# Zehong-Ma/MagCache

Measured on NVIDIA H100. Metric: denoising_steps_per_sec, higher is better.
Workload: dtype bf16

## Files before the change

### magcache_b200/csrc/attn_wgmma.cu

```cuda
#include <cstdlib>

#include "common.cuh"
#include "ptx.cuh"
#include "tma_host.cuh"

#ifndef MC_ATTN_EMU_DEFAULT
#define MC_ATTN_EMU_DEFAULT 0
#endif

namespace mc {

constexpr int kHD = 128;
constexpr int kLongMinLk = 1024;

struct AttnParams {
  int Lq, Lk, heads;
  int q_blocks, full_units, tail_units, tail_split;
  float* part_o;
  float2* part_ml;
  float scale_log2;
  __nv_bfloat16* out;
  int64_t ldo;
  int tile_rot;
  const uint32_t* seg_flags;
  const uint32_t* seg_epoch;
  int seg_rows;
};

struct WorkItem {
  int q_block, head;
  int split, nsplit;
  int tail_unit;
};

__device__ __forceinline__ WorkItem work_item(const AttnParams& p) {
  WorkItem w;
  int c = blockIdx.x, unit;
  if (c < p.full_units) {
    unit = c, w.split = 0, w.nsplit = 1, w.tail_unit = 0;
  } else {
    c -= p.full_units;
    w.tail_unit = c / p.tail_split;
    w.split = c - w.tail_unit * p.tail_split;
    w.nsplit = p.tail_split;
    unit = p.full_units + w.tail_unit;
  }
  w.head = unit / p.q_blocks;
  w.q_block = unit - w.head * p.q_blocks;
  return w;
}

template <uint32_t EMU_MASK>
__device__ __forceinline__ float exp2_sel(float x, int group) {
  return ((EMU_MASK >> (group & 7)) & 1u) ? ptx::ex2_emul(x) : ptx::ex2_approx(x);
}

__device__ __forceinline__ void wait_segments(const AttnParams& p, int row0, int rows) {
  if (p.seg_flags == nullptr) return;
  const uint32_t want = *reinterpret_cast<const volatile uint32_t*>(p.seg_epoch);
  const int last = min(row0 + rows, p.Lk) - 1;
  const int s0 = row0 / p.seg_rows, s1 = last / p.seg_rows;
  for (int s = s0; s <= s1; ++s) {
    const uint32_t* f = p.seg_flags + s;
    const long long t0 = clock64();
    for (;;) {
      uint32_t v;
      asm volatile("ld.acquire.sys.global.u32 %0, [%1];" : "=r"(v) : "l"(f) : "memory");
      if (static_cast<int32_t>(v - want) >= 0) break;
      __nanosleep(100);
      if (clock64() - t0 > MC_MBAR_TIMEOUT_CYCLES) {
        MC_DIAG("attention: key segment %d never arrived (flag %u, epoch %u)\n", s, v, want);
        __trap();
      }
    }
  }
  asm volatile("fence.proxy.async;" ::: "memory");
}

namespace ak {
constexpr int kBQ = 128;
constexpr int kQBytes = kBQ * kHD * 2;
constexpr int kThreads = 384;
constexpr int kProducerRegs = 24, kConsumerRegs = 240;
template <int BKV>
struct Layout {
  static constexpr int kKBytes = BKV * kHD * 2;
  static constexpr int kVBytes = BKV * kHD * 2;
  static constexpr int kOffK = kQBytes;
  static constexpr int kOffV = kOffK + 2 * kKBytes;
  static constexpr int kOffBar = kOffV + 2 * kVBytes;
  static constexpr int kSmem = kOffBar + 128;
};
}

template <int BKV, uint32_t EMU_MASK>
__global__ void __launch_bounds__(ak::kThreads, 1)
    attn_kernel(const __grid_constant__ CUtensorMap tmap_q, const __grid_constant__ CUtensorMap tmap_k,
                const __grid_constant__ CUtensorMap tmap_v, const AttnParams p) {
  using namespace ak;
  using L = Layout<BKV>;
  extern __shared__ __align__(1024) uint8_t smem[];
  uint64_t* bars = reinterpret_cast<uint64_t*>(smem + L::kOffBar);
  uint64_t* q_full = bars + 0;
  uint64_t* k_full = bars + 1;
  uint64_t* k_empty = bars + 3;
  uint64_t* v_full = bars + 5;
  uint64_t* v_empty = bars + 7;

  const int warp = threadIdx.x >> 5, lane = threadIdx.x & 31;
  const WorkItem wi = work_item(p);
  const int q0 = wi.q_block * kBQ;
  const int head = wi.head;
  const int total_tiles = (p.Lk + BKV - 1) / BKV;
  const int per_split = (total_tiles + wi.nsplit - 1) / wi.nsplit;
  const int t0 = wi.split * per_split;
  const int n_tiles = min(per_split, total_tiles - t0);
  auto tile_of = [&](int j) {
    int t = p.tile_rot + t0 + j;
    return t >= total_tiles ? t - total_tiles : t;
  };

  if (threadIdx.x == 0) {
    if ((ptx::smem_u32(smem) & 1023u) != 0) {
      MC_DIAG("attn_kernel: dynamic smem base not 1024-aligned\n");
      __trap();
    }
    ptx::prefetch_tmap(&tmap_q);
    ptx::prefetch_tmap(&tmap_k);
    ptx::prefetch_tmap(&tmap_v);
    ptx::mbar_init(q_full, 1);
    for (int s = 0; s < 2; ++s) {
      ptx::mbar_init(&k_full[s], 1);
      ptx::mbar_init(&k_empty[s], 8);
      ptx::mbar_init(&v_full[s], 1);
      ptx::mbar_init(&v_empty[s], 8);
    }
    ptx::fence_mbar_init();
  }
  __syncthreads();

  if (warp < 4) {
    ptx::setmaxnreg_dec<kProducerRegs>();
    if (warp == 0) {
      if (ptx::elect_one()) {
        ptx::mbar_expect_tx(q_full, kQBytes);
        ptx::tma_load_2d(smem, &tmap_q, q_full, head * kHD, q0);
        ptx::tma_load_2d(smem + kQBytes / 2, &tmap_q, q_full, head * kHD + 64, q0);
      }
      __syncwarp();
      for (int j = 0; j < n_tiles; ++j) {
        const int s = j & 1;
        const uint32_t ph = (j >> 1) & 1;
        const int kv0 = tile_of(j) * BKV;
        if (p.seg_flags != nullptr) {
          if (lane == 0) wait_segments(p, kv0, BKV);
          __syncwarp();
        }
        ptx::mbar_wait(&k_empty[s], ph ^ 1);
        if (ptx::elect_one()) {
          ptx::mbar_expect_tx(&k_full[s], L::kKBytes);
          ptx::tma_load_2d(smem + L::kOffK + s * L::kKBytes, &tmap_k, &k_full[s], head * kHD, kv0);
          ptx::tma_load_2d(smem + L::kOffK + s * L::kKBytes + L::kKBytes / 2, &tmap_k, &k_full[s], head * kHD + 64, kv0);
        }
        __syncwarp();
        ptx::mbar_wait(&v_empty[s], ph ^ 1);
        if (ptx::elect_one()) {
          ptx::mbar_expect_tx(&v_full[s], L::kVBytes);
          ptx::tma_load_2d(smem + L::kOffV + s * L::kVBytes, &tmap_v, &v_full[s], head * kHD, kv0);
          ptx::tma_load_2d(smem + L::kOffV + s * L::kVBytes + L::kVBytes / 2, &tmap_v, &v_full[s], head * kHD + 64, kv0);
        }
        __syncwarp();
      }
    }
  } else {
    ptx::setmaxnreg_inc<kConsumerRegs>();
    const int wg = (warp >> 2) - 1;
    const int r = wg * 64 + (warp & 3) * 16 + (lane >> 2);
    const int cq = 2 * (lane & 3);
    const uint32_t q_base = ptx::smem_u32(smem) + wg * (64 * 128);
    const uint32_t k_base = ptx::smem_u32(smem + L::kOffK), v_base = ptx::smem_u32(smem + L::kOffV);
    int j_ragged = -1;
    if (p.Lk % BKV != 0) {
      int jr = total_tiles - 1 - p.tile_rot - t0;
      if (jr < 0) jr += total_tiles;
      if (jr < n_tiles) j_ragged = jr;
    }
    float o[kHD / 2];
#pragma unroll
    for (int i = 0; i < kHD / 2; ++i) o[i] = 0.f;
    float m0 = -INFINITY, m1 = -INFINITY, l0 = 0.f, l1 = 0.f;
    bool timed_out = false;
    ptx::mbar_wait_or_flag(q_full, 0, timed_out);

    constexpr uint32_t kTurnThreads = 256;
    const uint32_t bar_own = 1 + wg, bar_other = 2 - wg;
    auto turn_begin = [&] { ptx::named_bar_sync(bar_own, kTurnThreads); };
    auto turn_end = [&] { ptx::named_bar_arrive(bar_other, kTurnThreads); };
    if (wg == 0) ptx::named_bar_arrive(bar_own, kTurnThreads);

    float sc[BKV / 2];
    uint32_t pa[BKV / 16][4];
    const int valid = p.Lk - (total_tiles - 1) * BKV;
    auto issue_s = [&](int j) {
      const int s = j & 1;
      ptx::wgmma_fence();
#pragma unroll
      for (int kk = 0; kk < kHD / 16; ++kk) {
        const uint64_t da = ptx::gmma_desc_sw128_kmajor(q_base + (kk >> 2) * (kQBytes / 2)) + 2 * (kk & 3);
        const uint64_t db = ptx::gmma_desc_sw128_kmajor(k_base + s * L::kKBytes + (kk >> 2) * (L::kKBytes / 2)) + 2 * (kk & 3);
        if constexpr (BKV == 128) {
          ptx::wgmma_m64n128k16_ss(sc, da, db, kk != 0 ? 1u : 0u);
        } else {
          ptx::wgmma_m64n64k16_ss(sc, da, db, kk != 0 ? 1u : 0u);
        }
      }
      ptx::wgmma_commit();
    };
    auto issue_pv = [&](int j) {
      const int s = j & 1;
      ptx::fence_regs(o);
      ptx::wgmma_fence();
      const uint64_t dv = ptx::gmma_desc_sw128_mnmajor(v_base + s * L::kVBytes, BKV * 128);
#pragma unroll
      for (int kk = 0; kk < BKV / 16; ++kk)
        ptx::wgmma_m64n128k16_rs_tb(o, pa[kk], dv + static_cast<uint64_t>(kk * (2048 / 16)), 1u);
      ptx::wgmma_commit();
    };
    auto softmax = [&](int j, float& f0, float& f1) {
      ptx::fence_regs(sc);
      __syncwarp();
      if (lane == 0) ptx::mbar_arrive(&k_empty[j & 1]);
      if (j == j_ragged) {
#pragma unroll
        for (int i = 0; i < BKV / 8; ++i)
#pragma unroll
          for (int e = 0; e < 4; ++e)
            if (8 * i + cq + (e & 1) >= valid) sc[4 * i + e] = -INFINITY;
      }
      float mx0 = -INFINITY, mx1 = -INFINITY;
#pragma unroll
      for (int i = 0; i < BKV / 8; ++i) {
        mx0 = fmaxf(mx0, fmaxf(sc[4 * i], sc[4 * i + 1]));
        mx1 = fmaxf(mx1, fmaxf(sc[4 * i + 2], sc[4 * i + 3]));
      }
#pragma unroll
      for (int off = 1; off <= 2; off <<= 1) {
        mx0 = fmaxf(mx0, __shfl_xor_sync(0xffffffffu, mx0, off));
        mx1 = fmaxf(mx1, __shfl_xor_sync(0xffffffffu, mx1, off));
      }
      const float mn0 = fmaxf(m0, mx0 * p.scale_log2), mn1 = fmaxf(m1, mx1 * p.scale_log2);
      f0 = ptx::ex2_approx(m0 - mn0), f1 = ptx::ex2_approx(m1 - mn1);
      m0 = mn0, m1 = mn1;
      l0 *= f0, l1 *= f1;
#pragma unroll
      for (int i = 0; i < BKV / 8; ++i) {
        sc[4 * i] = exp2_sel<EMU_MASK>(fmaf(sc[4 * i], p.scale_log2, -m0), i);
        sc[4 * i + 1] = exp2_sel<EMU_MASK>(fmaf(sc[4 * i + 1], p.scale_log2, -m0), i);
        sc[4 * i + 2] = exp2_sel<EMU_MASK>(fmaf(sc[4 * i + 2], p.scale_log2, -m1), i);
        sc[4 * i + 3] = exp2_sel<EMU_MASK>(fmaf(sc[4 * i + 3], p.scale_log2, -m1), i);
        l0 += sc[4 * i] + sc[4 * i + 1];
        l1 += sc[4 * i + 2] + sc[4 * i + 3];
      }
    };
    auto pack_p = [&] {
#pragma unroll
      for (int i = 0; i < BKV / 8; ++i) {
        pa[i >> 1][(i & 1) * 2] = pack_bf16x2(sc[4 * i], sc[4 * i + 1]);
        pa[i >> 1][(i & 1) * 2 + 1] = pack_bf16x2(sc[4 * i + 2], sc[4 * i + 3]);
      }
    };
    auto release_v = [&](int j) {
      ptx::fence_regs(o);
      __syncwarp();
      if (lane == 0) ptx::mbar_arrive(&v_empty[j & 1]);
    };
    auto rescale_o = [&](float f0, float f1) {
#pragma unroll
      for (int i = 0; i < kHD / 8; ++i) {
        o[4 * i] *= f0, o[4 * i + 1] *= f0;
        o[4 * i + 2] *= f1, o[4 * i + 3] *= f1;
      }
    };
    {
      ptx::mbar_wait_or_flag(&k_full[0], 0, timed_out);
      turn_begin();
      issue_s(0);
      turn_end();
      ptx::wgmma_wait<0>();
      float f0, f1;
      softmax(0, f0, f1);
      rescale_o(f0, f1);
      pack_p();
    }
    for (int j = 1; j < n_tiles; ++j) {
      ptx::mbar_wait_or_flag(&k_full[j & 1], (j >> 1) & 1, timed_out);
      ptx::mbar_wait_or_flag(&v_full[(j - 1) & 1], ((j - 1) >> 1) & 1, timed_out);
      turn_begin();
      issue_s(j);
      issue_pv(j - 1);
      turn_end();
      ptx::wgmma_wait<1>();
      float f0, f1;
      softmax(j, f0, f1);
      ptx::wgmma_wait<0>();
      release_v(j - 1);
      rescale_o(f0, f1);
      pack_p();
    }
    {
      const int j = n_tiles - 1;
      ptx::mbar_wait_or_flag(&v_full[j & 1], (j >> 1) & 1, timed_out);
      turn_begin();
      issue_pv(j);
      if (wg == 0) turn_end();
      ptx::wgmma_wait<0>();
      release_v(j);
    }
    if (timed_out) __trap();

#pragma unroll
    for (int off = 1; off <= 2; off <<= 1) {
      l0 += __shfl_xor_sync(0xffffffffu, l0, off);
      l1 += __shfl_xor_sync(0xffffffffu, l1, off);
    }
    const bool partial = wi.nsplit > 1;
#pragma unroll
    for (int h = 0; h < 2; ++h) {
      const float inv_l = 1.0f / (h ? l1 : l0);
      const int rt = r + 8 * h;
      const int row = q0 + rt;
      if (row >= p.Lq) continue;
      if (partial) {
        const int64_t prow = (static_cast<int64_t>(wi.split) * p.tail_units + wi.tail_unit) * kBQ + rt;
        if ((lane & 3) == 0) p.part_ml[prow] = make_float2(h ? m1 : m0, h ? l1 : l0);
        float* dst = p.part_o + prow * kHD + cq;
#pragma unroll
        for (int i = 0; i < kHD / 8; ++i)
          *reinterpret_cast<float2*>(dst + 8 * i) = make_float2(o[4 * i + 2 * h] * inv_l, o[4 * i + 2 * h + 1] * inv_l);
      } else {
        __nv_bfloat16* dst = p.out + static_cast<int64_t>(row) * p.ldo + head * kHD + cq;
#pragma unroll
        for (int i = 0; i < kHD / 8; ++i)
          *reinterpret_cast<uint32_t*>(dst + 8 * i) = pack_bf16x2(o[4 * i + 2 * h] * inv_l, o[4 * i + 2 * h + 1] * inv_l);
      }
    }
  }
}

__global__ void __launch_bounds__(256) attn_combine_kernel(const float* __restrict__ part_o, const float2* __restrict__ part_ml, int nsplit,
                                                           int tail_units, int full_units, int q_blocks, int rows_per_cta, int Lq,
                                                           __nv_bfloat16* __restrict__ out, int64_t ldo) {
  constexpr int kGroups = kHD / 8;
  const int64_t total = static_cast<int64_t>(tail_units) * rows_per_cta * kGroups;
  const int64_t split_stride = static_cast<int64_t>(tail_units) * rows_per_cta;
  for (int64_t i = static_cast<int64_t>(blockIdx.x) * blockDim.x + threadIdx.x; i < total; i += static_cast<int64_t>(gridDim.x) * blockDim.x) {
    const int64_t prow = i / kGroups;
    const int g = static_cast<int>(i - prow * kGroups);
    const int tu = static_cast<int>(prow / rows_per_cta), r = static_cast<int>(prow - static_cast<int64_t>(tu) * rows_per_cta);
    const int unit = full_units + tu;
    const int head = unit / q_blocks, row = (unit - head * q_blocks) * rows_per_cta + r;
    if (row >= Lq) continue;
    float mmax = -INFINITY;
    for (int s = 0; s < nsplit; ++s) mmax = fmaxf(mmax, part_ml[s * split_stride + prow].x);
    float acc[8] = {0.f, 0.f, 0.f, 0.f, 0.f, 0.f, 0.f, 0.f};
    float wsum = 0.f;
    for (int s = 0; s < nsplit; ++s) {
      const float2 ml = part_ml[s * split_stride + prow];
      const float w = ml.y * ptx::ex2_approx(ml.x - mmax);
      wsum += w;
      float v[8];
      ptx::ld_nc_v8_f32(part_o + (s * split_stride + prow) * kHD + g * 8, v);
#pragma unroll
      for (int j = 0; j < 8; ++j) acc[j] = fmaf(w, v[j], acc[j]);
    }
    const float inv = 1.0f / wsum;
#pragma unroll
    for (int j = 0; j < 8; ++j) acc[j] *= inv;
    *reinterpret_cast<uint4*>(out + static_cast<int64_t>(row) * ldo + head * kHD + g * 8) = pack_bf16x8(acc);
  }
}

struct AttnPlan {
  bool long_kernel;
  int q_blocks, kv_tile, total_tiles, rows_per_cta;
  int full_units, tail_units, tail_split;
  size_t ws_bytes;
  int grid() const { return full_units + tail_units * tail_split; }
};

static int env_int(const char* name, int lo, int hi, int dflt) {
  const char* e = getenv(name);
  if (!e || !*e) return dflt;
  const int v = atoi(e);
  return (v < lo || v > hi) ? dflt : v;
}

static AttnPlan plan_attention(int Lq, int Lk, int heads, bool need_long = false) {
  AttnPlan pl;
  const int forced_splits = env_int("MC_ATTN_SPLITS", 1, 16, 0);
  const int kernel_sel = env_int("MC_ATTN_KERNEL", 0, 2, 0);
  pl.long_kernel = need_long || kernel_sel == 2 || (kernel_sel == 0 && Lk >= kLongMinLk);
  pl.rows_per_cta = ak::kBQ;
  pl.kv_tile = pl.long_kernel ? 128 : 64;
  pl.q_blocks = (Lq + pl.rows_per_cta - 1) / pl.rows_per_cta;
  pl.total_tiles = (Lk + pl.kv_tile - 1) / pl.kv_tile;
  const int64_t units = static_cast<int64_t>(pl.q_blocks) * heads;
  const int slots = num_sms();
  const int min_tiles_per_split = pl.long_kernel ? 4 : 8;
  int full = static_cast<int>(units), tail = 0, split = 1;
  if (forced_splits > 0) {
    if (forced_splits > 1) full = 0, tail = static_cast<int>(units), split = forced_splits;
  } else {
    const int rem = static_cast<int>(units % slots);
    const int by_tiles = pl.total_tiles / min_tiles_per_split;
    int f = rem > 0 ? slots / rem : 1;
    if (f > 8) f = 8;
    if (f > by_tiles) f = by_tiles;
    if (f >= 2) full = static_cast<int>(units) - rem, tail = rem, split = f;
  }
  if (split > pl.total_tiles) split = pl.total_tiles;
  if (split > 1) {
    const int per = (pl.total_tiles + split - 1) / split;
    split = (pl.total_tiles + per - 1) / per;
  }
  if (split <= 1) full = static_cast<int>(units), tail = 0, split = 1;
  pl.full_units = full, pl.tail_units = tail, pl.tail_split = split;
  pl.ws_bytes = tail > 0 ? static_cast<size_t>(split) * tail * pl.rows_per_cta * (kHD * sizeof(float) + sizeof(float2)) : 0;
  return pl;
}

}

extern "C" int32_t mc_attn_workspace_bytes(int32_t Lq, int32_t Lk, int32_t heads, int64_t* bytes_out) {
  MC_CHECK_ARG(bytes_out != nullptr && Lq >= 1 && Lk >= 1 && heads >= 1, "mc_attn_workspace_bytes: bad arguments");
  const size_t a = mc::plan_attention(Lq, Lk, heads, false).ws_bytes, b = mc::plan_attention(Lq, Lk, heads, true).ws_bytes;
  *bytes_out = static_cast<int64_t>(a > b ? a : b);
  return MC_OK;
}

extern "C" int32_t mc_attn_fwd_ex(const void* q, int64_t ldq, const void* k, int64_t ldk, const void* v, int64_t ldv, void* out,
                                  int64_t ldo, int32_t Lq, int32_t Lk, int32_t heads, float scale, void* workspace,
                                  int64_t workspace_bytes, int32_t first_key_row, const uint32_t* seg_flags, const uint32_t* seg_epoch,
                                  int32_t seg_rows, void* stream) {
  MC_CHECK_ARG(q && k && v && out, "mc_attn_fwd: null pointer");
  MC_CHECK_ARG(Lq >= 1 && Lk >= 1 && heads >= 1, "mc_attn_fwd: Lq=%d Lk=%d heads=%d", Lq, Lk, heads);
  const int64_t width = static_cast<int64_t>(heads) * mc::kHD;
  MC_CHECK_ARG(ldq >= width && ldk >= width && ldo >= width && ldv >= width, "mc_attn_fwd: leading dimensions too small");
  MC_CHECK_ARG(ldq % 8 == 0 && ldk % 8 == 0 && ldv % 8 == 0 && ldo % 8 == 0, "mc_attn_fwd: leading dimensions must be multiples of 8");
  MC_CHECK_ARG(mc::aligned16(q) && mc::aligned16(k) && mc::aligned16(v) && mc::aligned16(out), "mc_attn_fwd: pointers must be 16-byte aligned");
  MC_CHECK_ARG(first_key_row >= 0 && first_key_row < Lk, "mc_attn_fwd: first_key_row=%d outside [0, %d)", first_key_row, Lk);
  MC_CHECK_ARG(seg_flags == nullptr || (seg_rows >= 1 && seg_epoch != nullptr), "mc_attn_fwd: seg_rows=%d / null epoch", seg_rows);
  const mc::AttnPlan pl = mc::plan_attention(Lq, Lk, heads, first_key_row != 0 || seg_flags != nullptr);
  MC_CHECK_ARG(static_cast<int64_t>(pl.q_blocks) * heads * 8 < INT32_MAX, "mc_attn_fwd: grid too large");
  if (pl.tail_units > 0) {
    MC_CHECK_ARG(workspace != nullptr && workspace_bytes >= static_cast<int64_t>(pl.ws_bytes) && (reinterpret_cast<uintptr_t>(workspace) & 31u) == 0,
                 "mc_attn_fwd: split-KV needs a 32-byte aligned workspace of %lld bytes (mc_attn_workspace_bytes), got %lld",
                 static_cast<long long>(pl.ws_bytes), static_cast<long long>(workspace_bytes));
  }
  const int q_box = mc::ak::kBQ;
  CUtensorMap tq, tk, tv;
  int32_t rc = mc::make_tmap_bf16_2d(&tq, q, static_cast<uint64_t>(Lq), static_cast<uint64_t>(width), static_cast<uint64_t>(ldq), q_box, 64);
  if (rc) return rc;
  rc = mc::make_tmap_bf16_2d(&tk, k, static_cast<uint64_t>(Lk), static_cast<uint64_t>(width), static_cast<uint64_t>(ldk), pl.kv_tile, 64);
  if (rc) return rc;
  rc = mc::make_tmap_bf16_2d(&tv, v, static_cast<uint64_t>(Lk), static_cast<uint64_t>(width), static_cast<uint64_t>(ldv), pl.kv_tile, 64);
  if (rc) return rc;

  float* part_o = static_cast<float*>(workspace);
  const size_t part_rows = static_cast<size_t>(pl.tail_split) * pl.tail_units * pl.rows_per_cta;
  float2* part_ml = pl.tail_units > 0 ? reinterpret_cast<float2*>(part_o + part_rows * mc::kHD) : nullptr;
  mc::AttnParams p{};
  p.Lq = Lq, p.Lk = Lk, p.heads = heads;
  p.q_blocks = pl.q_blocks, p.full_units = pl.full_units, p.tail_units = pl.tail_units, p.tail_split = pl.tail_split;
  p.part_o = pl.tail_units > 0 ? part_o : nullptr, p.part_ml = part_ml;
  p.scale_log2 = scale * 1.4426950408889634f;
  p.out = static_cast<__nv_bfloat16*>(out), p.ldo = ldo;
  p.tile_rot = ((first_key_row + pl.kv_tile - 1) / pl.kv_tile) % pl.total_tiles;
  p.seg_flags = seg_flags, p.seg_epoch = seg_epoch, p.seg_rows = seg_rows > 0 ? seg_rows : Lk;

  dim3 grid(pl.grid(), 1, 1);
  cudaStream_t st = static_cast<cudaStream_t>(stream);
  if (pl.long_kernel) {
    static mc::PerDeviceOnce once[4];
    const int emu = mc::env_int("MC_ATTN_EMU", 0, 4, MC_ATTN_EMU_DEFAULT);
#define MC_LAUNCH_LONG(MASK, IDX)                                                                                                    \
  do {                                                                                                                               \
    rc = mc::set_max_smem_once(mc::attn_kernel<128, MASK>, mc::ak::Layout<128>::kSmem, once[IDX], "cudaFuncSetAttribute(attn smem)"); \
    if (rc) return rc;                                                                                                               \
    mc::attn_kernel<128, MASK><<<grid, mc::ak::kThreads, mc::ak::Layout<128>::kSmem, st>>>(tq, tk, tv, p);                           \
  } while (0)
    switch (emu) {
      case 2: MC_LAUNCH_LONG(0x88u, 1); break;
      case 3: MC_LAUNCH_LONG(0x92u, 2); break;
      case 4: MC_LAUNCH_LONG(0xAAu, 3); break;
      default: MC_LAUNCH_LONG(0x00u, 0); break;
    }
#undef MC_LAUNCH_LONG
  } else {
    static mc::PerDeviceOnce once;
    rc = mc::set_max_smem_once(mc::attn_kernel<64, 0u>, mc::ak::Layout<64>::kSmem, once, "cudaFuncSetAttribute(attn smem)");
    if (rc) return rc;
    mc::attn_kernel<64, 0u><<<grid, mc::ak::kThreads, mc::ak::Layout<64>::kSmem, st>>>(tq, tk, tv, p);
  }
  MC_CHECK_LAUNCH("attn_kernel launch");
  if (pl.tail_units > 0) {
    const int64_t total = static_cast<int64_t>(pl.tail_units) * pl.rows_per_cta * (mc::kHD / 8);
    const int64_t want = (total + 255) / 256, cap = static_cast<int64_t>(mc::num_sms()) * 8;
    mc::attn_combine_kernel<<<static_cast<int>(want < cap ? want : cap), 256, 0, st>>>(
        p.part_o, p.part_ml, pl.tail_split, pl.tail_units, pl.full_units, pl.q_blocks, pl.rows_per_cta, Lq, static_cast<__nv_bfloat16*>(out), ldo);
    MC_CHECK_LAUNCH("attn_combine_kernel launch");
  }
  return MC_OK;
}

extern "C" int32_t mc_attn_fwd(const void* q, int64_t ldq, const void* k, int64_t ldk, const void* v, int64_t ldv, void* out,
                               int64_t ldo, int32_t Lq, int32_t Lk, int32_t heads, float scale, void* workspace,
                               int64_t workspace_bytes, void* stream) {
  return mc_attn_fwd_ex(q, ldq, k, ldk, v, ldv, out, ldo, Lq, Lk, heads, scale, workspace, workspace_bytes, 0, nullptr, nullptr, 0, stream);
}
```

Before: 1.654.

## Multicast K/V tiles across 2-CTA clusters in long attention kernel

The long-sequence attention kernel now runs as 2-CTA clusters that handle adjacent query blocks of the same head. Each CTA loads half of every K/V tile and multicasts it to both CTAs via TMA, and empty barriers are released cluster-wide. This halves L2-to-SM K/V traffic per query block. The ring also grows to three stages, and scheduling slots are sized with cudaOccupancyMaxActiveClusters. The cost is cross-CTA synchronisation coupling, since one slow CTA stalls its partner, plus coarser work units that can hurt load balance.

```diff
diff --git a/magcache_b200/csrc/attn_wgmma.cu b/magcache_b200/csrc/attn_wgmma.cu
--- a/magcache_b200/csrc/attn_wgmma.cu
+++ b/magcache_b200/csrc/attn_wgmma.cu
@@ -15,7 +15,7 @@
 
 struct AttnParams {
   int Lq, Lk, heads;
-  int q_blocks, full_units, tail_units, tail_split;
+  int head_units, full_units, tail_units, tail_split;
   float* part_o;
   float2* part_ml;
   float scale_log2;
@@ -33,9 +33,10 @@
   int tail_unit;
 };
 
-__device__ __forceinline__ WorkItem work_item(const AttnParams& p) {
+template <int CL>
+__device__ __forceinline__ WorkItem work_item(const AttnParams& p, int rank) {
   WorkItem w;
-  int c = blockIdx.x, unit;
+  int c = static_cast<int>(blockIdx.x / CL), unit;
   if (c < p.full_units) {
     unit = c, w.split = 0, w.nsplit = 1, w.tail_unit = 0;
   } else {
@@ -45,8 +46,8 @@
     w.nsplit = p.tail_split;
     unit = p.full_units + w.tail_unit;
   }
-  w.head = unit / p.q_blocks;
-  w.q_block = unit - w.head * p.q_blocks;
+  w.head = unit / p.head_units;
+  w.q_block = (unit - w.head * p.head_units) * CL + rank;
   return w;
 }
 
@@ -82,33 +83,40 @@
 constexpr int kQBytes = kBQ * kHD * 2;
 constexpr int kThreads = 384;
 constexpr int kProducerRegs = 24, kConsumerRegs = 240;
-template <int BKV>
+constexpr int kPairStages = 3;
+template <int BKV, int CL>
 struct Layout {
+  static constexpr int kStages = CL > 1 ? kPairStages : 2;
   static constexpr int kKBytes = BKV * kHD * 2;
   static constexpr int kVBytes = BKV * kHD * 2;
+  static constexpr int kPartRows = BKV / CL;
   static constexpr int kOffK = kQBytes;
-  static constexpr int kOffV = kOffK + 2 * kKBytes;
-  static constexpr int kOffBar = kOffV + 2 * kVBytes;
+  static constexpr int kOffV = kOffK + kStages * kKBytes;
+  static constexpr int kOffBar = kOffV + kStages * kVBytes;
   static constexpr int kSmem = kOffBar + 128;
 };
-}
-
-template <int BKV, uint32_t EMU_MASK>
+#define MC_RING_STAGE(S, j) ((S) == 2 ? ((j) & 1) : ((j) % (S)))
+#define MC_RING_PHASE(S, j) ((S) == 2 ? (((j) >> 1) & 1) : (((j) / (S)) & 1))
+}
+
+template <int BKV, uint32_t EMU_MASK, int CL>
 __global__ void __launch_bounds__(ak::kThreads, 1)
     attn_kernel(const __grid_constant__ CUtensorMap tmap_q, const __grid_constant__ CUtensorMap tmap_k,
                 const __grid_constant__ CUtensorMap tmap_v, const AttnParams p) {
   using namespace ak;
-  using L = Layout<BKV>;
+  using L = Layout<BKV, CL>;
+  constexpr int S = L::kStages;
   extern __shared__ __align__(1024) uint8_t smem[];
   uint64_t* bars = reinterpret_cast<uint64_t*>(smem + L::kOffBar);
   uint64_t* q_full = bars + 0;
   uint64_t* k_full = bars + 1;
-  uint64_t* k_empty = bars + 3;
-  uint64_t* v_full = bars + 5;
-  uint64_t* v_empty = bars + 7;
+  uint64_t* k_empty = bars + 1 + S;
+  uint64_t* v_full = bars + 1 + 2 * S;
+  uint64_t* v_empty = bars + 1 + 3 * S;
 
   const int warp = threadIdx.x >> 5, lane = threadIdx.x & 31;
-  const WorkItem wi = work_item(p);
+  const int rank = CL > 1 ? static_cast<int>(ptx::cluster_ctarank()) : 0;
+  const WorkItem wi = work_item<CL>(p, rank);
   const int q0 = wi.q_block * kBQ;
   const int head = wi.head;
   const int total_tiles = (p.Lk + BKV - 1) / BKV;
@@ -129,15 +137,20 @@
     ptx::prefetch_tmap(&tmap_k);
     ptx::prefetch_tmap(&tmap_v);
     ptx::mbar_init(q_full, 1);
-    for (int s = 0; s < 2; ++s) {
+    for (int s = 0; s < S; ++s) {
       ptx::mbar_init(&k_full[s], 1);
-      ptx::mbar_init(&k_empty[s], 8);
+      ptx::mbar_init(&k_empty[s], 8 * CL);
       ptx::mbar_init(&v_full[s], 1);
-      ptx::mbar_init(&v_empty[s], 8);
+      ptx::mbar_init(&v_empty[s], 8 * CL);
     }
     ptx::fence_mbar_init();
   }
-  __syncthreads();
+  if constexpr (CL > 1) {
+    ptx::cluster_arrive();
+    ptx::cluster_wait();
+  } else {
+    __syncthreads();
+  }
 
   if (warp < 4) {
     ptx::setmaxnreg_dec<kProducerRegs>();
@@ -149,27 +162,45 @@
       }
       __syncwarp();
       for (int j = 0; j < n_tiles; ++j) {
-        const int s = j & 1;
-        const uint32_t ph = (j >> 1) & 1;
+        const int s = MC_RING_STAGE(S, j);
+        const uint32_t ph = MC_RING_PHASE(S, j);
         const int kv0 = tile_of(j) * BKV;
-        if (p.seg_flags != nullptr) {
-          if (lane == 0) wait_segments(p, kv0, BKV);
+        if constexpr (CL == 1) {
+          if (p.seg_flags != nullptr) {
+            if (lane == 0) wait_segments(p, kv0, BKV);
+            __syncwarp();
+          }
+          ptx::mbar_wait(&k_empty[s], ph ^ 1);
+          if (ptx::elect_one()) {
+            ptx::mbar_expect_tx(&k_full[s], L::kKBytes);
+            ptx::tma_load_2d(smem + L::kOffK + s * L::kKBytes, &tmap_k, &k_full[s], head * kHD, kv0);
+            ptx::tma_load_2d(smem + L::kOffK + s * L::kKBytes + L::kKBytes / 2, &tmap_k, &k_full[s], head * kHD + 64, kv0);
+          }
+          __syncwarp();
+          ptx::mbar_wait(&v_empty[s], ph ^ 1);
+          if (ptx::elect_one()) {
+            ptx::mbar_expect_tx(&v_full[s], L::kVBytes);
+            ptx::tma_load_2d(smem + L::kOffV + s * L::kVBytes, &tmap_v, &v_full[s], head * kHD, kv0);
+            ptx::tma_load_2d(smem + L::kOffV + s * L::kVBytes + L::kVBytes / 2, &tmap_v, &v_full[s], head * kHD + 64, kv0);
+          }
+          __syncwarp();
+        } else {
+          const int kr = kv0 + rank * L::kPartRows;
+          const uint32_t off = static_cast<uint32_t>(rank) * (L::kPartRows * 128);
+          constexpr uint16_t kAll = static_cast<uint16_t>((1u << CL) - 1);
+          auto load_part = [&](const CUtensorMap* tmap, uint64_t* full, uint8_t* tile, int bytes) {
+            wait_segments(p, kr, L::kPartRows);
+            ptx::mbar_expect_tx(full, bytes);
+            ptx::tma_load_2d_multicast(tile + off, tmap, full, head * kHD, kr, kAll);
+            ptx::tma_load_2d_multicast(tile + bytes / 2 + off, tmap, full, head * kHD + 64, kr, kAll);
+          };
+          ptx::mbar_wait(&k_empty[s], ph ^ 1);
+          if (ptx::elect_one()) load_part(&tmap_k, &k_full[s], smem + L::kOffK + s * L::kKBytes, L::kKBytes);
+          __syncwarp();
+          ptx::mbar_wait(&v_empty[s], ph ^ 1);
+          if (ptx::elect_one()) load_part(&tmap_v, &v_full[s], smem + L::kOffV + s * L::kVBytes, L::kVBytes);
           __syncwarp();
         }
-        ptx::mbar_wait(&k_empty[s], ph ^ 1);
-        if (ptx::elect_one()) {
-          ptx::mbar_expect_tx(&k_full[s], L::kKBytes);
-          ptx::tma_load_2d(smem + L::kOffK + s * L::kKBytes, &tmap_k, &k_full[s], head * kHD, kv0);
-          ptx::tma_load_2d(smem + L::kOffK + s * L::kKBytes + L::kKBytes / 2, &tmap_k, &k_full[s], head * kHD + 64, kv0);
-        }
-        __syncwarp();
-        ptx::mbar_wait(&v_empty[s], ph ^ 1);
-        if (ptx::elect_one()) {
-          ptx::mbar_expect_tx(&v_full[s], L::kVBytes);
-          ptx::tma_load_2d(smem + L::kOffV + s * L::kVBytes, &tmap_v, &v_full[s], head * kHD, kv0);
-          ptx::tma_load_2d(smem + L::kOffV + s * L::kVBytes + L::kVBytes / 2, &tmap_v, &v_full[s], head * kHD + 64, kv0);
-        }
-        __syncwarp();
       }
     }
   } else {
@@ -202,7 +233,7 @@
     uint32_t pa[BKV / 16][4];
     const int valid = p.Lk - (total_tiles - 1) * BKV;
     auto issue_s = [&](int j) {
-      const int s = j & 1;
+      const int s = MC_RING_STAGE(S, j);
       ptx::wgmma_fence();
 #pragma unroll
       for (int kk = 0; kk < kHD / 16; ++kk) {
@@ -217,7 +248,7 @@
       ptx::wgmma_commit();
     };
     auto issue_pv = [&](int j) {
-      const int s = j & 1;
+      const int s = MC_RING_STAGE(S, j);
       ptx::fence_regs(o);
       ptx::wgmma_fence();
       const uint64_t dv = ptx::gmma_desc_sw128_mnmajor(v_base + s * L::kVBytes, BKV * 128);
@@ -226,10 +257,18 @@
         ptx::wgmma_m64n128k16_rs_tb(o, pa[kk], dv + static_cast<uint64_t>(kk * (2048 / 16)), 1u);
       ptx::wgmma_commit();
     };
+    auto release = [&](uint64_t* empty) {
+      if constexpr (CL > 1) {
+#pragma unroll
+        for (uint32_t c = 0; c < CL; ++c) ptx::mbar_arrive_cluster(empty, c);
+      } else {
+        ptx::mbar_arrive(empty);
+      }
+    };
     auto softmax = [&](int j, float& f0, float& f1) {
       ptx::fence_regs(sc);
       __syncwarp();
-      if (lane == 0) ptx::mbar_arrive(&k_empty[j & 1]);
+      if (lane == 0) release(&k_empty[MC_RING_STAGE(S, j)]);
       if (j == j_ragged) {
 #pragma unroll
         for (int i = 0; i < BKV / 8; ++i)
@@ -272,7 +311,7 @@
     auto release_v = [&](int j) {
       ptx::fence_regs(o);
       __syncwarp();
-      if (lane == 0) ptx::mbar_arrive(&v_empty[j & 1]);
+      if (lane == 0) release(&v_empty[MC_RING_STAGE(S, j)]);
     };
     auto rescale_o = [&](float f0, float f1) {
 #pragma unroll
@@ -293,8 +332,8 @@
       pack_p();
     }
     for (int j = 1; j < n_tiles; ++j) {
-      ptx::mbar_wait_or_flag(&k_full[j & 1], (j >> 1) & 1, timed_out);
-      ptx::mbar_wait_or_flag(&v_full[(j - 1) & 1], ((j - 1) >> 1) & 1, timed_out);
+      ptx::mbar_wait_or_flag(&k_full[MC_RING_STAGE(S, j)], MC_RING_PHASE(S, j), timed_out);
+      ptx::mbar_wait_or_flag(&v_full[MC_RING_STAGE(S, j - 1)], MC_RING_PHASE(S, j - 1), timed_out);
       turn_begin();
       issue_s(j);
       issue_pv(j - 1);
@@ -309,7 +348,7 @@
     }
     {
       const int j = n_tiles - 1;
-      ptx::mbar_wait_or_flag(&v_full[j & 1], (j >> 1) & 1, timed_out);
+      ptx::mbar_wait_or_flag(&v_full[MC_RING_STAGE(S, j)], MC_RING_PHASE(S, j), timed_out);
       turn_begin();
       issue_pv(j);
       if (wg == 0) turn_end();
@@ -331,7 +370,7 @@
       const int row = q0 + rt;
       if (row >= p.Lq) continue;
       if (partial) {
-        const int64_t prow = (static_cast<int64_t>(wi.split) * p.tail_units + wi.tail_unit) * kBQ + rt;
+        const int64_t prow = (static_cast<int64_t>(wi.split) * p.tail_units + wi.tail_unit) * (CL * kBQ) + rank * kBQ + rt;
         if ((lane & 3) == 0) p.part_ml[prow] = make_float2(h ? m1 : m0, h ? l1 : l0);
         float* dst = p.part_o + prow * kHD + cq;
 #pragma unroll
@@ -345,20 +384,24 @@
       }
     }
   }
+  if constexpr (CL > 1) {
+    ptx::cluster_arrive();
+    ptx::cluster_wait();
+  }
 }
 
 __global__ void __launch_bounds__(256) attn_combine_kernel(const float* __restrict__ part_o, const float2* __restrict__ part_ml, int nsplit,
-                                                           int tail_units, int full_units, int q_blocks, int rows_per_cta, int Lq,
+                                                           int tail_units, int full_units, int head_units, int unit_rows, int Lq,
                                                            __nv_bfloat16* __restrict__ out, int64_t ldo) {
   constexpr int kGroups = kHD / 8;
-  const int64_t total = static_cast<int64_t>(tail_units) * rows_per_cta * kGroups;
-  const int64_t split_stride = static_cast<int64_t>(tail_units) * rows_per_cta;
+  const int64_t total = static_cast<int64_t>(tail_units) * unit_rows * kGroups;
+  const int64_t split_stride = static_cast<int64_t>(tail_units) * unit_rows;
   for (int64_t i = static_cast<int64_t>(blockIdx.x) * blockDim.x + threadIdx.x; i < total; i += static_cast<int64_t>(gridDim.x) * blockDim.x) {
     const int64_t prow = i / kGroups;
     const int g = static_cast<int>(i - prow * kGroups);
-    const int tu = static_cast<int>(prow / rows_per_cta), r = static_cast<int>(prow - static_cast<int64_t>(tu) * rows_per_cta);
+    const int tu = static_cast<int>(prow / unit_rows), r = static_cast<int>(prow - static_cast<int64_t>(tu) * unit_rows);
     const int unit = full_units + tu;
-    const int head = unit / q_blocks, row = (unit - head * q_blocks) * rows_per_cta + r;
+    const int head = unit / head_units, row = (unit - head * head_units) * unit_rows + r;
     if (row >= Lq) continue;
     float mmax = -INFINITY;
     for (int s = 0; s < nsplit; ++s) mmax = fmaxf(mmax, part_ml[s * split_stride + prow].x);
@@ -380,13 +423,53 @@
   }
 }
 
+constexpr int kLongCluster = 2;
+
 struct AttnPlan {
   bool long_kernel;
-  int q_blocks, kv_tile, total_tiles, rows_per_cta;
+  int cluster;
+  int head_units, kv_tile, total_tiles, unit_rows;
   int full_units, tail_units, tail_split;
   size_t ws_bytes;
-  int grid() const { return full_units + tail_units * tail_split; }
+  int grid() const { return cluster * (full_units + tail_units * tail_split); }
 };
+
+static int32_t long_kernel_slots(int* out) {
+  static int cached[kMaxDevices] = {};
+  const int d = current_device();
+  if (cached[d] > 0) {
+    *out = cached[d];
+    return MC_OK;
+  }
+  int devices = 0;
+  if (cudaGetDeviceCount(&devices) != cudaSuccess || devices == 0) {
+    (void)cudaGetLastError();
+    *out = num_sms() / kLongCluster;
+    return MC_OK;
+  }
+  static PerDeviceOnce once;
+  constexpr int kSmem = ak::Layout<128, kLongCluster>::kSmem;
+  int32_t rc = set_max_smem_once(attn_kernel<128, 0u, kLongCluster>, kSmem, once, "cudaFuncSetAttribute(attn smem)");
+  if (rc) return rc;
+  cudaLaunchAttribute attr[1];
+  attr[0].id = cudaLaunchAttributeClusterDimension;
+  attr[0].val.clusterDim.x = kLongCluster, attr[0].val.clusterDim.y = 1, attr[0].val.clusterDim.z = 1;
+  cudaLaunchConfig_t cfg = {};
+  cfg.gridDim = dim3(kLongCluster * num_sms(), 1, 1);
+  cfg.blockDim = dim3(ak::kThreads, 1, 1);
+  cfg.dynamicSmemBytes = kSmem;
+  cfg.attrs = attr, cfg.numAttrs = 1;
+  int n = 0;
+  const cudaError_t e = cudaOccupancyMaxActiveClusters(&n, attn_kernel<128, 0u, kLongCluster>, &cfg);
+  if (e != cudaSuccess) return cuda_fail(e, "cudaOccupancyMaxActiveClusters(attn)");
+  if (n < 1) {
+    set_error("attn_kernel: no cluster of %d CTAs with %d B of shared memory fits on this device", kLongCluster, kSmem);
+    return MC_ERR_CUDA;
+  }
+  cached[d] = n;
+  *out = n;
+  return MC_OK;
+}
 
 static int env_int(const char* name, int lo, int hi, int dflt) {
   const char* e = getenv(name);
@@ -395,17 +478,22 @@
   return (v < lo || v > hi) ? dflt : v;
 }
 
-static AttnPlan plan_attention(int Lq, int Lk, int heads, bool need_long = false) {
+static int32_t plan_attention(int Lq, int Lk, int heads, bool need_long, AttnPlan* out) {
   AttnPlan pl;
   const int forced_splits = env_int("MC_ATTN_SPLITS", 1, 16, 0);
   const int kernel_sel = env_int("MC_ATTN_KERNEL", 0, 2, 0);
   pl.long_kernel = need_long || kernel_sel == 2 || (kernel_sel == 0 && Lk >= kLongMinLk);
-  pl.rows_per_cta = ak::kBQ;
+  pl.cluster = pl.long_kernel ? kLongCluster : 1;
+  pl.unit_rows = pl.cluster * ak::kBQ;
   pl.kv_tile = pl.long_kernel ? 128 : 64;
-  pl.q_blocks = (Lq + pl.rows_per_cta - 1) / pl.rows_per_cta;
+  pl.head_units = (Lq + pl.unit_rows - 1) / pl.unit_rows;
   pl.total_tiles = (Lk + pl.kv_tile - 1) / pl.kv_tile;
-  const int64_t units = static_cast<int64_t>(pl.q_blocks) * heads;
-  const int slots = num_sms();
+  const int64_t units = static_cast<int64_t>(pl.head_units) * heads;
+  int slots = num_sms();
+  if (pl.long_kernel) {
+    const int32_t rc = long_kernel_slots(&slots);
+    if (rc) return rc;
+  }
   const int min_tiles_per_split = pl.long_kernel ? 4 : 8;
   int full = static_cast<int>(units), tail = 0, split = 1;
   if (forced_splits > 0) {
@@ -425,16 +513,41 @@
   }
   if (split <= 1) full = static_cast<int>(units), tail = 0, split = 1;
   pl.full_units = full, pl.tail_units = tail, pl.tail_split = split;
-  pl.ws_bytes = tail > 0 ? static_cast<size_t>(split) * tail * pl.rows_per_cta * (kHD * sizeof(float) + sizeof(float2)) : 0;
-  return pl;
+  pl.ws_bytes = tail > 0 ? static_cast<size_t>(split) * tail * pl.unit_rows * (kHD * sizeof(float) + sizeof(float2)) : 0;
+  *out = pl;
+  return MC_OK;
+}
+
+template <uint32_t MASK>
+static int32_t launch_attn_long(dim3 grid, const CUtensorMap& tq, const CUtensorMap& tk, const CUtensorMap& tv, const AttnParams& p,
+                                cudaStream_t st, PerDeviceOnce& once) {
+  constexpr int kSmem = ak::Layout<128, kLongCluster>::kSmem;
+  int32_t rc = set_max_smem_once(attn_kernel<128, MASK, kLongCluster>, kSmem, once, "cudaFuncSetAttribute(attn smem)");
+  if (rc) return rc;
+  cudaLaunchAttribute attr[1];
+  attr[0].id = cudaLaunchAttributeClusterDimension;
+  attr[0].val.clusterDim.x = kLongCluster, attr[0].val.clusterDim.y = 1, attr[0].val.clusterDim.z = 1;
+  cudaLaunchConfig_t cfg = {};
+  cfg.gridDim = grid;
+  cfg.blockDim = dim3(ak::kThreads, 1, 1);
+  cfg.dynamicSmemBytes = kSmem;
+  cfg.stream = st;
+  cfg.attrs = attr, cfg.numAttrs = 1;
+  const cudaError_t e = cudaLaunchKernelEx(&cfg, attn_kernel<128, MASK, kLongCluster>, tq, tk, tv, p);
+  if (e != cudaSuccess) return cuda_fail(e, "attn_kernel launch");
+  return MC_OK;
 }
 
 }
 
 extern "C" int32_t mc_attn_workspace_bytes(int32_t Lq, int32_t Lk, int32_t heads, int64_t* bytes_out) {
   MC_CHECK_ARG(bytes_out != nullptr && Lq >= 1 && Lk >= 1 && heads >= 1, "mc_attn_workspace_bytes: bad arguments");
-  const size_t a = mc::plan_attention(Lq, Lk, heads, false).ws_bytes, b = mc::plan_attention(Lq, Lk, heads, true).ws_bytes;
-  *bytes_out = static_cast<int64_t>(a > b ? a : b);
+  mc::AttnPlan a, b;
+  int32_t rc = mc::plan_attention(Lq, Lk, heads, false, &a);
+  if (rc) return rc;
+  rc = mc::plan_attention(Lq, Lk, heads, true, &b);
+  if (rc) return rc;
+  *bytes_out = static_cast<int64_t>(a.ws_bytes > b.ws_bytes ? a.ws_bytes : b.ws_bytes);
   return MC_OK;
 }
 
@@ -450,8 +563,10 @@
   MC_CHECK_ARG(mc::aligned16(q) && mc::aligned16(k) && mc::aligned16(v) && mc::aligned16(out), "mc_attn_fwd: pointers must be 16-byte aligned");
   MC_CHECK_ARG(first_key_row >= 0 && first_key_row < Lk, "mc_attn_fwd: first_key_row=%d outside [0, %d)", first_key_row, Lk);
   MC_CHECK_ARG(seg_flags == nullptr || (seg_rows >= 1 && seg_epoch != nullptr), "mc_attn_fwd: seg_rows=%d / null epoch", seg_rows);
-  const mc::AttnPlan pl = mc::plan_attention(Lq, Lk, heads, first_key_row != 0 || seg_flags != nullptr);
-  MC_CHECK_ARG(static_cast<int64_t>(pl.q_blocks) * heads * 8 < INT32_MAX, "mc_attn_fwd: grid too large");
+  mc::AttnPlan pl;
+  int32_t rc = mc::plan_attention(Lq, Lk, heads, first_key_row != 0 || seg_flags != nullptr, &pl);
+  if (rc) return rc;
+  MC_CHECK_ARG(static_cast<int64_t>(pl.head_units) * pl.cluster * heads * 8 < INT32_MAX, "mc_attn_fwd: grid too large");
   if (pl.tail_units > 0) {
     MC_CHECK_ARG(workspace != nullptr && workspace_bytes >= static_cast<int64_t>(pl.ws_bytes) && (reinterpret_cast<uintptr_t>(workspace) & 31u) == 0,
                  "mc_attn_fwd: split-KV needs a 32-byte aligned workspace of %lld bytes (mc_attn_workspace_bytes), got %lld",
@@ -459,19 +574,20 @@
   }
   const int q_box = mc::ak::kBQ;
   CUtensorMap tq, tk, tv;
-  int32_t rc = mc::make_tmap_bf16_2d(&tq, q, static_cast<uint64_t>(Lq), static_cast<uint64_t>(width), static_cast<uint64_t>(ldq), q_box, 64);
-  if (rc) return rc;
-  rc = mc::make_tmap_bf16_2d(&tk, k, static_cast<uint64_t>(Lk), static_cast<uint64_t>(width), static_cast<uint64_t>(ldk), pl.kv_tile, 64);
-  if (rc) return rc;
-  rc = mc::make_tmap_bf16_2d(&tv, v, static_cast<uint64_t>(Lk), static_cast<uint64_t>(width), static_cast<uint64_t>(ldv), pl.kv_tile, 64);
+  rc = mc::make_tmap_bf16_2d(&tq, q, static_cast<uint64_t>(Lq), static_cast<uint64_t>(width), static_cast<uint64_t>(ldq), q_box, 64);
+  if (rc) return rc;
+  const int kv_box = pl.kv_tile / pl.cluster;
+  rc = mc::make_tmap_bf16_2d(&tk, k, static_cast<uint64_t>(Lk), static_cast<uint64_t>(width), static_cast<uint64_t>(ldk), kv_box, 64);
+  if (rc) return rc;
+  rc = mc::make_tmap_bf16_2d(&tv, v, static_cast<uint64_t>(Lk), static_cast<uint64_t>(width), static_cast<uint64_t>(ldv), kv_box, 64);
   if (rc) return rc;
 
   float* part_o = static_cast<float*>(workspace);
-  const size_t part_rows = static_cast<size_t>(pl.tail_split) * pl.tail_units * pl.rows_per_cta;
+  const size_t part_rows = static_cast<size_t>(pl.tail_split) * pl.tail_units * pl.unit_rows;
   float2* part_ml = pl.tail_units > 0 ? reinterpret_cast<float2*>(part_o + part_rows * mc::kHD) : nullptr;
   mc::AttnParams p{};
   p.Lq = Lq, p.Lk = Lk, p.heads = heads;
-  p.q_blocks = pl.q_blocks, p.full_units = pl.full_units, p.tail_units = pl.tail_units, p.tail_split = pl.tail_split;
+  p.head_units = pl.head_units, p.full_units = pl.full_units, p.tail_units = pl.tail_units, p.tail_split = pl.tail_split;
   p.part_o = pl.tail_units > 0 ? part_o : nullptr, p.part_ml = part_ml;
   p.scale_log2 = scale * 1.4426950408889634f;
   p.out = static_cast<__nv_bfloat16*>(out), p.ldo = ldo;
@@ -483,31 +599,25 @@
   if (pl.long_kernel) {
     static mc::PerDeviceOnce once[4];
     const int emu = mc::env_int("MC_ATTN_EMU", 0, 4, MC_ATTN_EMU_DEFAULT);
-#define MC_LAUNCH_LONG(MASK, IDX)                                                                                                    \
-  do {                                                                                                                               \
-    rc = mc::set_max_smem_once(mc::attn_kernel<128, MASK>, mc::ak::Layout<128>::kSmem, once[IDX], "cudaFuncSetAttribute(attn smem)"); \
-    if (rc) return rc;                                                                                                               \
-    mc::attn_kernel<128, MASK><<<grid, mc::ak::kThreads, mc::ak::Layout<128>::kSmem, st>>>(tq, tk, tv, p);                           \
-  } while (0)
     switch (emu) {
-      case 2: MC_LAUNCH_LONG(0x88u, 1); break;
-      case 3: MC_LAUNCH_LONG(0x92u, 2); break;
-      case 4: MC_LAUNCH_LONG(0xAAu, 3); break;
-      default: MC_LAUNCH_LONG(0x00u, 0); break;
-    }
-#undef MC_LAUNCH_LONG
+      case 2: rc = mc::launch_attn_long<0x88u>(grid, tq, tk, tv, p, st, once[1]); break;
+      case 3: rc = mc::launch_attn_long<0x92u>(grid, tq, tk, tv, p, st, once[2]); break;
+      case 4: rc = mc::launch_attn_long<0xAAu>(grid, tq, tk, tv, p, st, once[3]); break;
+      default: rc = mc::launch_attn_long<0x00u>(grid, tq, tk, tv, p, st, once[0]); break;
+    }
+    if (rc) return rc;
   } else {
     static mc::PerDeviceOnce once;
-    rc = mc::set_max_smem_once(mc::attn_kernel<64, 0u>, mc::ak::Layout<64>::kSmem, once, "cudaFuncSetAttribute(attn smem)");
+    rc = mc::set_max_smem_once(mc::attn_kernel<64, 0u, 1>, mc::ak::Layout<64, 1>::kSmem, once, "cudaFuncSetAttribute(attn smem)");
     if (rc) return rc;
-    mc::attn_kernel<64, 0u><<<grid, mc::ak::kThreads, mc::ak::Layout<64>::kSmem, st>>>(tq, tk, tv, p);
-  }
-  MC_CHECK_LAUNCH("attn_kernel launch");
+    mc::attn_kernel<64, 0u, 1><<<grid, mc::ak::kThreads, mc::ak::Layout<64, 1>::kSmem, st>>>(tq, tk, tv, p);
+    MC_CHECK_LAUNCH("attn_kernel launch");
+  }
   if (pl.tail_units > 0) {
-    const int64_t total = static_cast<int64_t>(pl.tail_units) * pl.rows_per_cta * (mc::kHD / 8);
+    const int64_t total = static_cast<int64_t>(pl.tail_units) * pl.unit_rows * (mc::kHD / 8);
     const int64_t want = (total + 255) / 256, cap = static_cast<int64_t>(mc::num_sms()) * 8;
     mc::attn_combine_kernel<<<static_cast<int>(want < cap ? want : cap), 256, 0, st>>>(
-        p.part_o, p.part_ml, pl.tail_split, pl.tail_units, pl.full_units, pl.q_blocks, pl.rows_per_cta, Lq, static_cast<__nv_bfloat16*>(out), ldo);
+        p.part_o, p.part_ml, pl.tail_split, pl.tail_units, pl.full_units, pl.head_units, pl.unit_rows, Lq, static_cast<__nv_bfloat16*>(out), ldo);
     MC_CHECK_LAUNCH("attn_combine_kernel launch");
   }
   return MC_OK;
```

After: 1.677, median of 6. 1.01x the previous value.
